# Infinidat/slimfastq

Hardware: AMD Instinct MI355X
Metric: MB/s FASTQ compressed (higher is better)
Workload: dtype u8/u32 integer; 1 GPU; synthetic 10M x 150 bp Illumina reads per GPU, full qlts+gens+recs, frozen tables (one chain per lane), -l 3; level=3, block_reads=1024, prior_step=-1, blocks_per_gpu=9766, tables=frozen, chains_per_gpu=253906, raw_bytes_per_gpu=3702038404, parallelism=1 GPU

## Files before the change

slimfastq_amd/csrc/chains.hip:

```cpp
#include "kernels.h"
#include "dev_chain.h"
#include "dev_walk.h"
#include "dev_wave.h"
#include "gen_pack_place.h"
typedef u32 __attribute__((aligned(1))) u32_any;

#define LAST_QLT 63u
#define QROW_BYTES 256u
#define B2_INIT 0x03030303u

#define QDEC_ROW 72u
__device__ __forceinline__ void qdec_store(u16* row, u32 s, u32 cum) {
    if (s) row[8 + s - 1] = (u16)cum;
    if ((s & 7u) == 0) row[s >> 3] = (u16)cum;
    if (s == 63) row[8 + 63] = 0;
}
__global__ __launch_bounds__(256) void k_qlt_frozen_rows(const u32* __restrict__ rows66, u32 q_rows, u32* __restrict__ qrows, u16* __restrict__ qdec) {
    const u32 lane = threadIdx.x & 63;
    const u32 ctx = blockIdx.x * 4 + (threadIdx.x >> 6);
    if (ctx >= q_rows) return;
    const u32* r = rows66 + (size_t)ctx * 66;
    const u32 slot = r[lane], iend = r[65];
    if (iend == 0) {
        qrows[(size_t)ctx * 64 + lane] = (lane << 10) | (1024u << 16);
// ... 904 lines not shown
            const u32 rec = s0 + sub;
            uint4 e = tab[rec & 63u];
            if (rec >= n) e.w = 0;
            const u32 last = gp_step_last(s0, n, per);
            const u32 rec_end = done + rl(inc, last), last_len = rl(len, last);
            u32 q0 = 0;
            do {
                const u32 off = q0 + piece;
                if (off < e.w) {
                    const uint4 w = load16(buf, nbytes, ((u64)e.y << 32 | e.x) + off);
                    const uint4 vm = gp_valid4(e.w - off);
                    u32 o0, o1, o2, o3, i0, i1, i2, i3;
                    const u32 f0 = gp_fold(gp_codes(w.x, vm.x, o0, i0)), f1 = gp_fold(gp_codes(w.y, vm.y, o1, i1));
                    const u32 f2 = gp_fold(gp_codes(w.z, vm.z, o2, i2)), f3 = gp_fold(gp_codes(w.w, vm.w, o3, i3));
                    illegal |= i0 | i1 | i2 | i3;
                    u32 p01 = __builtin_amdgcn_perm(f1, f0, 0x06020400u), p23 = __builtin_amdgcn_perm(f3, f2, 0x06020400u);
                    p01 |= p01 >> 12; p23 |= p23 >> 12;
                    const u32 code = __builtin_amdgcn_perm(p23, p01, 0x05040100u);
                    if (a.exc_flag && (o0 | o1 | o2 | o3)) a.exc_flag[cp.r0 + k0 + rec] = 1;
                    const GpPlace g = gp_place(e.z + off, code);
                    __hip_atomic_fetch_or(&ring[gp_ring_slot(g.d)], g.lo, __ATOMIC_RELAXED, __HIP_MEMORY_SCOPE_WAVEFRONT);
                    __hip_atomic_fetch_or(&ring[gp_ring_slot(g.d + 1u)], g.hi, __ATOMIC_RELAXED, __HIP_MEMORY_SCOPE_WAVEFRONT);
                }
                const u32 next = gp_turn_end(rec_end, last_len, q0);
                gp_wave_fence();
                if (gp_row_ready(row, next)) {
                    const u32 t = row + lane, slot = gp_ring_slot(t);
                    const u32 v = ring[slot];
                    ring[slot] = 0;
                    if (4u * t < cap) out[t] = v;
                    row += GP_ROW;
                }
                gp_wave_fence();
                q0 += 1024u;
            } while (q0 < last_len);
        }
        done += rl(inc, 63u);
    }
    {
        const u32 t = row + lane;
        if (lane < gp_tail_dwords(row, done) && 4u * t < cap) out[t] = ring[gp_ring_slot(t)];
    }
    if (lane == 0) {
        const u32 n = (done + 3u) >> 2;
        a.csz[c] = n;
        if (n > cap) atomicMax(&a.m.blocks[cp.b].status, (u32)(-SFQ_E_OVERFLOW));
    }
    if (__any(illegal != 0u) && lane == 0) atomicMax(&a.m.blocks[cp.b].status, (u32)(-SFQ_E_GENCHAR));
}
void launch_gen_encode_c(const ChainArgs& a, hipStream_t st, u32 c0, u32 c1, bool flat) {
    constexpr int T = 256;
    if (!c1 || c1 > a.geo.nchains) c1 = a.geo.nchains;
    if (c1 <= c0) return;
    if (a.flat_raw) { hipLaunchKernelGGL(k_gen_pack_raw, dim3((c1 - c0 + 3) / 4), dim3(256), 0, st, a, c0, c1); return; }
    const dim3 grid((c1 - c0 + T - 1) / T);
    if (flat) hipLaunchKernelGGL((k_gen_encode_c<T, true>), grid, dim3(T), 0, st, a, c0, c1);
    else hipLaunchKernelGGL((k_gen_encode_c<T, false>), grid, dim3(T), 0, st, a, c0, c1);
}

__device__ __forceinline__ u32 b2_pick(u32 v, LaneDecQ& rc, const u32* rcp) {
    const u32 f0 = v & 0xff, f1 = (v >> 8) & 0xff, f2 = (v >> 16) & 0xff, f3 = v >> 24;
    const u32 c1 = f0, c2 = f0 + f1, c3 = c2 + f2, tot = c3 + f3;
    u32 r;
    const u32 prob = rc.get_freq(tot, rcp[tot], r);
    const u32 b = (prob >= c1 ? 1u : 0u) + (prob >= c2 ? 1u : 0u) + (prob >= c3 ? 1u : 0u);
    const u32 cum = b == 0 ? 0u : b == 1 ? c1 : b == 2 ? c2 : c3;
    rc.decode(r, cum, (v >> (8 * b)) & 0xff);
    return b;
}
template <int THREADS>
__global__ __launch_bounds__(THREADS) void k_gen_decode_c(ChainArgs a, DecodeArgs da, u32 c0, u32 c1 ) {
    __shared__ u32 rcp[1024];
    for (u32 i = threadIdx.x; i < 1024; i += THREADS) rcp[i] = i ? rc_recip(i) : 0u;
    __syncthreads();
    const u32 c = c0 + blockIdx.x * THREADS + threadIdx.x;
    if (c >= c1) return;
    ChainPos cp = chain_pos(a, c);
    const BlockDesc* d = &a.m.blocks[cp.b];
    LaneDecQ rc; rc.init(da.streams + a.coff[c], a.csz[c], reinterpret_cast<const u8*>(a.qesc));
    const u32* rows = gen_rows_of(a, cp.b);
    const u32 alphabet = d->solid ? 0x33323130u  : 0x54474341u ;
    const u32 mask = (1u << d->gen_bits) - 1u;
    const u32 INIT = 0x007616c7u;
    const u32 r12 = rc_recip(12u);
    u32 n_next = cp.nrec ? da.slen[cp.r0] : 0u; u64 off_next = cp.nrec ? da.soff[cp.r0] : 0ull;
    if (a.seg_len) {
        const u32 ql = da.qlen[cp.r0];
        seg_range(cp, ql > n_next ? ql : n_next);
        const u64 lo = cp.sub_lo < n_next ? cp.sub_lo : n_next;
        n_next = (u32)(n_next - lo < cp.sub_len ? n_next - lo : cp.sub_len); off_next += lo;
    }
    const u8* const raw = da.streams + a.coff[c]; const u32 raw_n = a.csz[c];
    u32 racc = 0, rnb = 0, rat = 0, rbad = 0;
    for (u32 k = 0; k < cp.nrec; k++) {
        const u32 llen = n_next; const u64 off = off_next;
        if (k + 1 < cp.nrec) { n_next = da.slen[cp.r0 + k + 1]; off_next = da.soff[cp.r0 + k + 1]; }
        LaneOut32 out; out.begin(da.seq_stage + off);
        u32 last = INIT;
        if (a.flat_raw) {
            for (u32 i = 0; i < llen; i++) {
                if (rnb == 0) {
                    if (rat + 4u <= raw_n) { racc = *reinterpret_cast<const u32_any*>(raw + rat); rat += 4u; rnb = 32u; }
                    else if (rat < raw_n) { racc = raw[rat++]; rnb = 8u; }
                    else { rbad = 1; racc = 0; rnb = 32u; }
                }
                out.put((alphabet >> (8u * (racc & 3u))) & 0xffu);
                racc >>= 2; rnb -= 2u;
            }
        } else
        if (rows) {
            u32 v = rows[last & mask];
            for (u32 i = 0; i < llen; i++) {
                const uint4 cand = *reinterpret_cast<const uint4*>(rows + ((last << 2) & mask));
                rc.top_up();
                const u32 b = b2_pick(v, rc, rcp);
                out.put((alphabet >> (8 * b)) & 0xff);
                last = (last << 2) | b;
                v = b == 0 ? cand.x : b == 1 ? cand.y : b == 2 ? cand.z : cand.w;
            }
        } else if (a.flat_quads) {
            for (u32 i = 0; i < llen; i += 4u) {
                const u32 k = llen - i < 4u ? llen - i : 4u;
                rc.top_up();
                u32 r;
                const u32 S = rc.get_freq_bits(2u * k, r);
                rc.decode1(r, S, 1u);
                for (u32 j = 0; j < k; j++) out.put((alphabet >> (8u * ((S >> (2u * j)) & 3u))) & 0xffu);
            }
        } else {
            for (u32 i = 0; i < llen; i++) {
                rc.top_up();
                u32 r;
                const u32 prob = rc.get_freq(12u, r12, r);
                const u32 b = (prob >= 3u ? 1u : 0u) + (prob >= 6u ? 1u : 0u) + (prob >= 9u ? 1u : 0u);
                rc.decode1(r, 3u * b, 3u);
                out.put((alphabet >> (8 * b)) & 0xff);
            }
        }
        out.end();
    }
    if (a.flat_raw) { if (rbad || rat != raw_n || (rnb >= 8u) || racc) atomicMax(&a.m.blocks[cp.b].status, (u32)(-SFQ_E_CORRUPT)); }
    else
    if (rc.err) atomicMax(&a.m.blocks[cp.b].status, (u32)(-SFQ_E_CORRUPT));
}
void launch_gen_decode_c(const ChainArgs& a, const DecodeArgs& da, u32 c0, u32 c1, hipStream_t st) {
    constexpr int T = 256;
    if (c1 > a.geo.nchains) c1 = a.geo.nchains;
    if (c1 <= c0) return;
    hipLaunchKernelGGL(k_gen_decode_c<T>, dim3((c1 - c0 + T - 1) / T), dim3(T), 0, st, a, da, c0, c1);
}

#include "dev_rec_lane.h"
#include "dev_wave.h"

struct RecChainPos { u32 b; u64 r0; u32 nrec; };
__device__ __forceinline__ RecChainPos rec_chain_pos(const ChainArgs& a, u32 c) {
    RecChainPos p;
    p.b = c / a.rgeo.cpb;
    const u32 j = c - p.b * a.rgeo.cpb;
    const BlockDesc* d = &a.m.blocks[p.b];
    const u32 k0 = j * a.rgeo.chain_reads;
    p.nrec = k0 < d->nrec ? (d->nrec - k0 < a.rgeo.chain_reads ? d->nrec - k0 : a.rgeo.chain_reads) : 0u;
    p.r0 = d->rec0 + k0;
    return p;
}
__device__ __forceinline__ u8* rec_chain_region(const ChainArgs& a, const RecChainPos& p, u32& cap) {
    const BlockDesc* d = &a.m.blocks[p.b];
    const u64 t0 = a.m.line_off[4 * d->rec0], tc = a.m.line_off[4 * p.r0], te = a.m.line_off[4 * (p.r0 + p.nrec)];
    const u64 lo = ((tc - t0) * 3 / 2 + 3) & ~3ull, hi = ((te - t0) * 3 / 2) & ~3ull;
    cap = hi > lo ? (u32)(hi - lo) : 0u;
    return a.m.arena + d->out_off[SFQ_S_REC] + lo;
}

#define REC_HBUF 128u
#define REC_LDS_ROWS 8u
struct RecFrozenEnc {
    static constexpr bool inband = true;
    const u32* rows; LaneEnc rc;
    u8* lbuf;
    const u16* lmap; const u32* lrows;
    __device__ __forceinline__ void record(u32) {}
    __device__ __forceinline__ const u8* stage(const u8* g, u32 n, u32 k) {
        if (n + 1 > REC_HBUF) return g;
        u8* dst = lbuf + (k & 1u) * REC_HBUF;
        const u32 nw = (n + 4) / 4;
#pragma unroll 8
        for (u32 i = 0; i < nw; i++) reinterpret_cast<u32*>(dst)[i] = reinterpret_cast<const u32_any*>(g)[i];
        return dst;
    }
    __device__ __forceinline__ void put(u32 row, u32 sym) {
        const u32 slot = lmap[row];
        const u32 e = slot != 0xFFFFu ? lrows[slot * 256 + sym] : rows[(size_t)row * 256 + sym];
        rc.encode16(FZ_CUM(e), FZ_FREQ(e));
    }
    __device__ __forceinline__ void put_u(u32 row0, u64 num) { put_u_rows(*this, row0, num); }
};
struct RecCountEnc {
    static constexpr bool inband = true;
    u32* cnt; u32 kc;
    __device__ __forceinline__ void record(u32 k) { kc = k; }
    __device__ __forceinline__ const u8* stage(const u8* g, u32, u32) { return g; }
    __device__ __forceinline__ void put(u32 row, u32 sym) { atomicAdd(&cnt[(size_t)row * 256 + sym], kc >= 1u ? 1u : 0u); }
    __device__ __forceinline__ void put_u(u32 row0, u64 num) { put_u_rows(*this, row0, num); }
};
__global__ __launch_bounds__(64) void k_rec_count(ModelArgs a, u64 nrec, u64 stride, u32 run, u32 nruns, u32* cnt, const u32* flags ) {
    const u32 i = blockIdx.x * 64 + threadIdx.x;
    if (i >= nruns) return;
    if (flags && !flags[i]) return;
    const u64 r0 = (u64)i * stride;
    if (r0 >= nrec) return;
    const u32 n = (u32)(nrec - r0 < run ? nrec - r0 : run);
    RecCountEnc cd; cd.cnt = cnt + (size_t)(blockIdx.x % REC_COUNT_COPIES) * PR_REC_ROWS * 256; cd.kc = 0;
    XfEnc x_rec; x_rec.init(nullptr, 0, XF_REC_X);
    PwTab none; none.slots = nullptr; none.hdr = nullptr; none.epoch = 0;
    u32 hb; int bad;
    rec_encode_lane(a, r0, r0, n, cd, x_rec, none, hb, bad);
}
__global__ __launch_bounds__(256) void k_rec_count_sum(u32* __restrict__ cnt) {
    const u32 i = blockIdx.x * 256 + threadIdx.x;
    if (i >= PR_REC_ROWS * 256u) return;
    u32 s = 0;
#pragma unroll 8
    for (u32 k = 1; k < REC_COUNT_COPIES; k++) s += cnt[(size_t)k * PR_REC_ROWS * 256 + i];
    if (s) cnt[i] += s;
}
#define RDEC_ROW 272u
__global__ __launch_bounds__(256) void k_rec_frozen_rows(const u32* __restrict__ f, u32 nrows, u32* __restrict__ rrows, u16* __restrict__ rdec) {
    const u32 lane = threadIdx.x & 63;
    const u32 row = blockIdx.x * 4 + (threadIdx.x >> 6);
    if (row >= nrows) return;
    const uint4 fv = *reinterpret_cast<const uint4*>(f + (size_t)row * 256 + lane * 4);
    const u32 x[4] = { fv.x + 1, fv.y + 1, fv.z + 1, fv.w + 1 };
    u32 S = x[0] + x[1] + x[2] + x[3];
#pragma unroll
    for (int d = 32; d > 0; d >>= 1) S += (u32)__shfl_xor((int)S, d, 64);
    u32 g[4]; u32 sum = 0, best = 0;
#pragma unroll
    for (int j = 0; j < 4; j++) {
        g[j] = (u32)(((u64)x[j] << 16) / S); g[j] = g[j] ? g[j] : 1u;
        sum += g[j];
        const u32 key = (g[j] << 8) | (255u - (lane * 4 + j));
        best = key > best ? key : best;
    }
#pragma unroll
    for (int d = 32; d > 0; d >>= 1) {
        sum += (u32)__shfl_xor((int)sum, d, 64);
        const u32 o = (u32)__shfl_xor((int)best, d, 64); best = o > best ? o : best;
    }
    const u32 bsym = 255u - (best & 255u);
#pragma unroll
    for (int j = 0; j < 4; j++) if (lane * 4 + j == bsym) g[j] += 65536u - sum;
    const u32 mine = g[0] + g[1] + g[2] + g[3];
    u32 incl = mine;
#pragma unroll
    for (int d = 1; d < 64; d <<= 1) { const u32 o = (u32)__shfl_up((int)incl, d, 64); if (lane >= (u32)d) incl += o; }
    u32 cum = incl - mine;
    if (rdec) {
        u16* rd = rdec + (size_t)row * RDEC_ROW;
        if ((lane & 3) == 0) rd[lane >> 2] = (u16)cum;
        const u32 c1 = cum + g[0], c2 = c1 + g[1], c3 = c2 + g[2];
        *reinterpret_cast<uint2*>(rd + 16 + lane * 4) = make_uint2(cum | (c1 << 16), c2 | (c3 << 16));
    }
    uint4 e;
    e.x = cum | (g[0] << 16); cum += g[0];
    e.y = cum | (g[1] << 16); cum += g[1];
    e.z = cum | (g[2] << 16); cum += g[2];
    e.w = cum | (g[3] << 16);
    *reinterpret_cast<uint4*>(rrows + (size_t)row * 256 + lane * 4) = e;
}
__global__ __launch_bounds__(256) void k_rec_prior_freqs(const u32* __restrict__ cnt, u32 nrows, u32* __restrict__ f, u32* __restrict__ rtot) {
    const u32 lane = threadIdx.x & 63;
    const u32 row = blockIdx.x * 4 + (threadIdx.x >> 6);
    if (row >= nrows) return;
    const uint4 cv = *reinterpret_cast<const uint4*>(cnt + (size_t)row * 256 + lane * 4);
    u32 mx = max(max(cv.x, cv.y), max(cv.z, cv.w));
#pragma unroll
    for (int d = 32; d > 0; d >>= 1) { const u32 o = (u32)__shfl_xor((int)mx, d, 64); mx = o > mx ? o : mx; }
    u32 sh = 0;
    while ((((u64)mx * 14u) >> sh) > 32000u) sh++;
    uint4 fv;
    fv.x = (u32)(((u64)cv.x * 14u) >> sh); fv.y = (u32)(((u64)cv.y * 14u) >> sh); fv.z = (u32)(((u64)cv.z * 14u) >> sh); fv.w = (u32)(((u64)cv.w * 14u) >> sh);
    *reinterpret_cast<uint4*>(f + (size_t)row * 256 + lane * 4) = fv;
    u32 t = fv.x + fv.y + fv.z + fv.w;
#pragma unroll
    for (int d = 32; d > 0; d >>= 1) t += (u32)__shfl_xor((int)t, d, 64);
    if (lane == 0) rtot[row] = t;
}
#define RHR_PER ((PR_REC_ROWS + 255u) / 256u)
__global__ __launch_bounds__(256) void k_rec_hot_rows(const u32* __restrict__ rtot, u32 nrows, u32 nh, u16* __restrict__ map, u16* __restrict__ hot) {
    __shared__ u64 wmax[4];
    const u32 t = threadIdx.x, lane = t & 63, wave = t >> 6;
    u64 k[RHR_PER];
#pragma unroll
    for (u32 j = 0; j < RHR_PER; j++) {
        const u32 row = t + 256u * j;
        k[j] = row < nrows ? ((u64)rtot[row] << 11) | (2047u - row) : 0ull;
        if (row < nrows) map[row] = 0xFFFFu;
    }
    for (u32 i = 0; i < nh; i++) {
        u64 m = 0;
#pragma unroll
        for (u32 j = 0; j < RHR_PER; j++) m = k[j] > m ? k[j] : m;
#pragma unroll
        for (int d = 32; d > 0; d >>= 1) {
            const u64 o = ((u64)(u32)__shfl_xor((int)(u32)(m >> 32), d, 64) << 32) | (u32)__shfl_xor((int)(u32)m, d, 64);
            m = o > m ? o : m;
// ... 152 lines not shown
            u32 type = nw_lds(L, cur, lane, o, (int)wl, fnum, pct);
            if (type != ST_STR && !rec_number_prints_back(type, wl, L.text[cur][o][lane])) type = ST_STR;
            const u32 rr = (f + 1) * 16;
            if (type == ST_STR) {
                cd.put(rr + 0, type);
                cd.put_u(rr + 2, wl);
                for (u32 j = 0; j < wl; j++) cd.put(rr + 1, L.text[cur][o + j][lane]);
                L.fkind[f][lane] = 0;
                continue;
            }
            const u64 was = pct ? L.fvalue[f][lane] : 0;
            u64 gap;
            L.fkind[f][lane] = (type < ST_STR || type >= ST_DGT_Z) ? 1 : 2;
            L.fvalue[f][lane] = fnum;
            if (fnum < was) { gap = was - fnum; type++; }
            else gap = fnum - was;
            cd.put(rr + 0, type);
            cd.put_u(rr + 2, gap);
        }
        nf_prev = nf; cur = prv;
    }
    hdr_bytes_out = hdr_bytes;
    return true;
}
template <u32 ML>
__global__ __launch_bounds__(64) void k_rec_encode_f(ChainArgs a, u32* flags, const u32* only ) {
    __builtin_amdgcn_s_setprio(3);
    __shared__ RecFastLds<ML> L;
    const u32 lane = threadIdx.x;
    {
        const u32 c0 = blockIdx.x * 64 + lane;
        if (only && !__any(c0 < a.rgeo.nchains && only[c0] == 1)) return;
    }
    for (u32 i = lane; i < PR_REC_ROWS; i += 64) { const u32 sl = a.rmap[i]; L.map[i] = (u8)(sl < REC_LDS_ROWS ? sl : 0xFFu); }
    for (u32 i = lane; i < a.r_hot * 256; i += 64) L.rows[i] = a.rrows[(size_t)a.rhot[i >> 8] * 256 + (i & 255)];
    __syncthreads();
    const u32 c = blockIdx.x * 64 + lane;
    if (c >= a.rgeo.nchains) return;
    if (only && !only[c]) return;
    const RecChainPos cp = rec_chain_pos(a, c);
    BlockDesc* d = &a.m.blocks[cp.b];
    u32 cap = 0;
    u8* outp = rec_chain_region(a, cp, cap);
    RecFastEnc<RecFastLds<ML>> cd; cd.rows = a.rrows; cd.L = &L; cd.rc.init(outp, cap);
    u32 hdr_bytes = 0;
    if (!rec_fast_lane(a.m, L, lane, d->rec0, cp.r0, cp.nrec, cd, hdr_bytes)) { flags[c] = 1; return; }
    a.rhb[c] = hdr_bytes;
    a.csz[c] = cd.rc.finish();
    if (cd.rc.err & 2) atomicMax(&d->status, (u32)(-SFQ_E_OVERFLOW));
    if (cd.rc.err & 1) atomicMax(&d->status, (u32)(-SFQ_E_CORRUPT));
}
struct RecFastCount {
    u32* cnt; u32 kc;
    __device__ __forceinline__ void record(u32 k) { kc = k; }
    __device__ __forceinline__ void put(u32 row, u32 sym) { atomicAdd(&cnt[(size_t)row * 256 + sym], kc >= 1u ? 1u : 0u); }
    __device__ __forceinline__ void put_u(u32 row0, u64 num) { put_u_rows(*this, row0, num); }
};
__global__ __launch_bounds__(64) void k_rec_count_f(ModelArgs a, u64 nrec, u64 stride, u32 run, u32 nruns, u32* cnt, u32* flags) {
    __shared__ RecFastLds<127> L;
    const u32 lane = threadIdx.x;
    const u32 i = blockIdx.x * 64 + lane;
    if (i >= nruns) return;
    const u64 r0 = (u64)i * stride;
    if (r0 >= nrec) return;
    const u32 n = (u32)(nrec - r0 < run ? nrec - r0 : run);
    bool fits = true;
    for (u32 k = 0; k < n && fits; k++) {
        const u64 h0 = a.line_off[4 * (r0 + k)] + 1, h1 = a.line_off[4 * (r0 + k) + 1] - 1;
        const u32 len = h1 > h0 ? (u32)(h1 - h0) : 0;
        fits = len <= 127u && rf_stage(L, 0, lane, a.fq + h0, len) <= RF_NF;
    }
    if (!fits) { flags[i] = 1; return; }
    RecFastCount cd; cd.cnt = cnt + (size_t)(blockIdx.x % REC_COUNT_COPIES) * PR_REC_ROWS * 256; cd.kc = 0;
    u32 hb = 0;
    rec_fast_lane(a, L, lane, r0, r0, n, cd, hb);
}
void launch_rec_count(const ModelArgs& a, u64 nrec, u64 stride, u32 run, u32 nruns, u32* cnt, u32* flags, hipStream_t st) {
    hipLaunchKernelGGL(k_rec_count_f, dim3((nruns + 63) / 64), dim3(64), 0, st, a, nrec, stride, run, nruns, cnt, flags);
    hipLaunchKernelGGL(k_rec_count, dim3((nruns + 63) / 64), dim3(64), 0, st, a, nrec, stride, run, nruns, cnt, (const u32*)flags);
    hipLaunchKernelGGL(k_rec_count_sum, dim3((PR_REC_ROWS * 256u + 255) / 256), dim3(256), 0, st, cnt);
}
#define RT_TOK_PER_REC 40u
#define RT_STAGED 24u
template <u32 ML>
struct RecTokLds {
    static constexpr u32 maxlen = ML;
    static constexpr u32 NW = (ML + 4) / 4;
    static constexpr u32 NWP = NW | 1u;
    u32 tw[66][NWP];
    u8 off[1][RF_NF][66], wln[1][RF_NF][66], sep[1][RF_NF][66];
    u8 nf[66];
    u32 tokst[RT_STAGED][64];
    __device__ __forceinline__ u32 byte(u32 col, u32 pos) const { return reinterpret_cast<const u8*>(tw[col])[pos]; }
};
struct HdrMask {
    u64 lo, hi;
    __device__ __forceinline__ u32 count() const { return (u32)__popcll(lo) + (u32)__popcll(hi); }
    __device__ __forceinline__ u32 take() {
        if (lo) { const u32 p = (u32)__ffsll((long long)lo) - 1u; lo &= lo - 1; return p; }
        const u32 p = 63u + (u32)__ffsll((long long)hi); hi &= hi - 1; return p;
    }
};
template <typename LT>
__device__ __forceinline__ bool rt_stage(LT& L, u32 col, const u8* text, u32 n, HdrMask& M) {
    const u32_any* g = reinterpret_cast<const u32_any*>(text);
    const u32 kn = n >> 2, nw = kn + 1;
    const u32 fill = (n & 3u) == 3u ? 0u : ~0u << (8u * ((n & 3u) + 1u));
    u32 zero = 0, mw[4] = {};
#pragma unroll
    for (u32 k0 = 0; k0 < LT::NW; k0 += 4) {
        if (!__any(k0 < nw)) break;
        u32 wv[4];
#pragma unroll
        for (u32 q = 0; q < 4; q++) wv[q] = k0 + q < nw && k0 + q < LT::NW ? g[k0 + q] : ~0u;
#pragma unroll
        for (u32 q = 0; q < 4; q++) {
            const u32 k = k0 + q;
            if (k >= LT::NW) break;
            L.tw[col][k] = wv[q];
            const u32 w = wv[q] | (k == kn ? fill : 0u);
            const u32 x = w & 0x7f7f7f7fu, y = x | 0x20202020u;
            const u32 dig = (x + 0x50505050u) & ~(x + 0x46464646u);
            const u32 let = (y + 0x1f1f1f1fu) & ~(y + 0x05050505u);
            const u32 t = ~((dig | let) & ~w) & 0x80808080u;
            mw[k / 8] |= (((t >> 7) * 0x01020408u) >> 24) << (4u * (k % 8));
            zero |= ~(((w & 0x7f7f7f7fu) + 0x7f7f7f7fu) | w) & 0x80808080u;
        }
    }
    M.lo = mw[0] | ((u64)mw[1] << 32);
    M.hi = mw[2] | ((u64)mw[3] << 32);
    if (n < 63) { M.lo &= (2ull << n) - 1; M.hi = 0; }
    else if (n == 63) M.hi = 0;
    else M.hi &= (2ull << (n - 64)) - 1;
    return zero == 0;
}
template <typename LT>
__device__ __forceinline__ void rt_fields(LT& L, u32 col, HdrMask m, u32 nf) {
    u32 start = 0;
    for (u32 f = 0; f < nf; f++) {
        const u32 p = m.take();
        L.off[0][f][col] = (u8)start; L.wln[0][f][col] = (u8)(p - start); L.sep[0][f][col] = (u8)L.byte(col, p);
        start = p + 1;
    }
}
struct TokCount { u32 n; __device__ __forceinline__ void put(u32, u32) { n++; } __device__ __forceinline__ void put_u(u32 row0, u64 num) { put_u_rows(*this, row0, num); } };
struct TokStage {
    u32* p; u32 n;
    __device__ __forceinline__ void put(u32 row, u32 sym) { if (n < RT_STAGED) p[n * 64u] = (row << 8) | sym; n++; }
    __device__ __forceinline__ void put_u(u32 row0, u64 num) { put_u_rows(*this, row0, num); }
};
struct TokStore { u32* p; __device__ __forceinline__ void put(u32 row, u32 sym) { *p++ = (row << 8) | sym; } __device__ __forceinline__ void put_u(u32 row0, u64 num) { put_u_rows(*this, row0, num); } };
template <typename LT>
__device__ __forceinline__ u32 nw_tok(const LT& L, u32 col, u32 off, u32 len, u64& num) {
    u32 v = 0, lead = 0;
    bool plain = len <= 9u;
    if (plain)
        for (u32 j = 0; j < len; j++) {
            const u32 d = L.byte(col, off + j) - '0';
            plain = plain && d <= 9u;
            lead |= (j < 2u && d == 0u) ? 1u << j : 0u;
            v = v * 10u + d;
        }
    if (plain) {
        num = (lead & 3u) == 3u ? 0u : v;
        return (lead & 3u) == 3u ? ST_STR : (lead & 1u) ? ST_DGT_Z : ST_DGT;
    }
    return field_type([&](u32 j) -> u32 { return L.byte(col, off + j); }, len, num, 0);
}
template <typename LT, typename EM>
__device__ __forceinline__ bool rec_tokens(const LT& L, u32 col, u32 n, u32 nf, bool shape, u64 map, u64 since, EM& em) {
    em.put(REC_FLAG_ROW, shape ? 1u : 0u);
    if (shape) {
        em.put_u(REC_FLAG_ROW + 2, n);
        for (u32 j = 0; j < n; j++) em.put(REC_FLAG_ROW + 1, L.byte(col, j));
        return true;
    }
    em.put_u(0 * 16 + 2, map);
    for (u64 todo = map; todo; todo &= todo - 1) {
        const u32 f = (u32)__ffsll((long long)todo) - 1u;
        const u32 o = L.off[0][f][col], wl = L.wln[0][f][col];
        u64 fnum;
        u32 type = nw_tok(L, col, o, wl, fnum);
        if (type != ST_STR && !rec_number_prints_back(type, wl, L.byte(col, o))) type = ST_STR;
        if (type >= ST_HGT && type <= ST_HLTC_Z) return false;
        const u32 rr = (f + 1) * 16;
        if (type == ST_STR) {
            em.put(rr + 0, type);
            em.put_u(rr + 2, wl);
            for (u32 j = 0; j < wl; j++) em.put(rr + 1, L.byte(col, o + j));
            continue;
        }
        u64 was = 0;
        if ((since >> f) & 1) {
            const u32 po = L.off[0][f][col - 1], pwl = L.wln[0][f][col - 1];
            u64 pn;
            u32 pt = nw_tok(L, col - 1, po, pwl, pn);
            if (pt != ST_STR && !rec_number_prints_back(pt, pwl, L.byte(col - 1, po))) pt = ST_STR;
            if (pt == ST_DGT || pt == ST_DGT_Z) was = pn;
        }
        u64 gap;
        if (fnum < was) { gap = was - fnum; type++; }
        else gap = fnum - was;
        em.put(rr + 0, type);
        em.put_u(rr + 2, gap);
    }
    return true;
}
template <u32 ML>
__global__ __launch_bounds__(64) void k_rec_tokens(ChainArgs a, u32* __restrict__ tok, u32* __restrict__ ntok, u32* __restrict__ flags) {
    __shared__ RecTokLds<ML> L;
    const u32 lane = threadIdx.x, col = lane + 1;
    const u32 c = blockIdx.x;
    const RecChainPos cp = rec_chain_pos(a, c);
    if (cp.nrec == 0) { if (lane == 0) { ntok[c] = 0; a.rhb[c] = 0; } return; }
    const u64 base = a.m.blocks[cp.b].rec0;
    u32 bad = 0, base_n = 0;
    if (lane == 0) {
        const u64 h0 = a.m.line_off[4 * base] + 1, h1 = a.m.line_off[4 * base + 1] - 1;
        base_n = h1 > h0 ? (u32)(h1 - h0) : 0;
        if (base_n > ML) bad = 1;
        else {
            HdrMask m0;
            const bool ok = rt_stage(L, 0, a.m.fq + h0, base_n, m0);
            const u32 nf = m0.count();
            if (!ok || nf > RF_NF) bad = 1; else { rt_fields(L, 0, m0, nf); L.nf[0] = (u8)nf; }
        }
    }
    if (__any(bad != 0)) { if (lane == 0) flags[c] = 1; return; }
    const u64 end = cp.r0 + cp.nrec;
    const u64 first = cp.r0 == base ? cp.r0 + 1 : cp.r0;
    u32 hdr_bytes = cp.r0 == base ? rl(base_n, 0) : 0u;
    u64 since0 = 0;
    u32 total = 0;
    u32* const out = tok + cp.r0 * RT_TOK_PER_REC;
    const u32 cap = cp.nrec * RT_TOK_PER_REC;
    for (u64 rb = first; rb < end; rb += 64) {
        const u64 r = rb + lane;
        const bool valid = r < end;
        u32 n = 0, nf = 0;
        if (valid) {
            const u64 h0 = a.m.line_off[4 * r] + 1, h1 = a.m.line_off[4 * r + 1] - 1;
            n = h1 > h0 ? (u32)(h1 - h0) : 0;
            if (n > ML) bad = 1;
            else {
                HdrMask m;
                const bool ok = rt_stage(L, col, a.m.fq + h0, n, m);
                nf = m.count();
                if (!ok || nf > RF_NF) bad = 1; else { rt_fields(L, col, m, nf); L.nf[col] = (u8)nf; }
            }
        }
        if (__any(bad != 0)) { if (lane == 0) flags[c] = 1; return; }
        __syncthreads();
        bool shape = false; u64 map = 0;
        if (valid) {
            shape = nf != L.nf[col - 1];
            for (u32 f = 0; !shape && f < nf; f++) shape = L.sep[0][f][col] != L.sep[0][f][col - 1];
            if (!shape)
                for (u32 f = 0; f < nf; f++) {
                    const u32 wl = L.wln[0][f][col];
                    bool ch = wl != L.wln[0][f][col - 1];
                    if (!ch) {
                        const u32 o = L.off[0][f][col], po = L.off[0][f][col - 1];
                        for (u32 j = 0; j < wl; j++) if (L.byte(col, o + j) != L.byte(col - 1, po + j)) { ch = true; break; }
                    }
                    if (ch) map |= 1ull << f;
                }
        }
        u32 rs = shape ? 1u : 0u; u64 mm = shape ? 0ull : map;
#pragma unroll
        for (u32 dd = 1; dd < 64; dd <<= 1) {
            const u32 ors = (u32)__shfl_up((int)rs, dd, 64);
            const u64 omm = (u64)__shfl_up((unsigned long long)mm, dd, 64);
            if (lane >= dd) { mm = rs ? mm : (mm | omm); rs |= ors; }
        }
        u32 ers = (u32)__shfl_up((int)rs, 1, 64); u64 emm = (u64)__shfl_up((unsigned long long)mm, 1, 64);
        if (lane == 0) { ers = 0; emm = 0; }
        const u64 since = ers ? emm : (since0 | emm);
        {
            const u32 lrs = (u32)__shfl((int)rs, 63, 64); const u64 lmm = (u64)__shfl((unsigned long long)mm, 63, 64);
            since0 = lrs ? lmm : (since0 | lmm);
        }
        TokStage tl; tl.p = &L.tokst[0][lane]; tl.n = 0;
        bool ok = true;
        if (valid) ok = rec_tokens(L, col, n, nf, shape, map, since, tl);
        if (__any(!ok)) { if (lane == 0) flags[c] = 1; return; }
        const u32 cnt = tl.n;
        const u32 incl = wave_incl_scan(cnt);
        const u32 round = rl(incl, 63);
        if (total + round > cap) { if (lane == 0) flags[c] = 1; return; }
        u32* const dst = out + total + (incl - cnt);
        if (__any(cnt > RT_STAGED)) {
            if (valid) { TokStore ts; ts.p = dst; rec_tokens(L, col, n, nf, shape, map, since, ts); }
        } else
            for (u32 j = 0; __any(j < cnt); j++) if (j < cnt) dst[j] = L.tokst[j][lane];
        total += round;
        hdr_bytes += rl(wave_incl_scan(n), 63);
        __syncthreads();
        if (rb + 64 < end) {
            for (u32 p = lane; p < RecTokLds<ML>::NWP; p += 64) L.tw[0][p] = L.tw[64][p];
            if (lane < RF_NF) { L.off[0][lane][0] = L.off[0][lane][64]; L.wln[0][lane][0] = L.wln[0][lane][64]; L.sep[0][lane][0] = L.sep[0][lane][64]; }
            if (lane == 0) L.nf[0] = L.nf[64];
            __syncthreads();
        }
    }
    if (lane == 0) { ntok[c] = total; a.rhb[c] = hdr_bytes; }
}
#define RC_LDS_ROWS 16u
struct RecCodeLds { u32 rows[RC_LDS_ROWS * 256]; u8 map[PR_REC_ROWS]; };
__device__ __forceinline__ u32 rec_code_entry(const RecCodeLds& L, const u32* __restrict__ grows, u32 row, u32 sym) {
    const u32 slot = L.map[row];
    return slot != 0xFFu ? L.rows[slot * 256 + sym] : grows[(size_t)row * 256 + sym];
}
__global__ __launch_bounds__(256) void k_rec_code(ChainArgs a, const u32* __restrict__ tok, const u32* __restrict__ ntok, const u32* __restrict__ flags, u32 n_hot) {
    __shared__ RecCodeLds L;
    for (u32 i = threadIdx.x; i < PR_REC_ROWS; i += 256) { const u32 sl = a.rmap[i]; L.map[i] = (u8)(sl < n_hot ? sl : 0xFFu); }
    for (u32 i = threadIdx.x; i < n_hot * 256; i += 256) L.rows[i] = a.rrows[(size_t)a.rhot[i >> 8] * 256 + (i & 255)];
    __syncthreads();
    const u32 c = blockIdx.x * 256 + threadIdx.x;
    if (c >= a.rgeo.nchains || flags[c]) return;
    const RecChainPos cp = rec_chain_pos(a, c);
    BlockDesc* d = &a.m.blocks[cp.b];
    u32 cap = 0;
    u8* outp = rec_chain_region(a, cp, cap);
    RecFastEnc<RecCodeLds> cd; cd.rows = a.rrows; cd.L = &L; cd.rc.init(outp, cap);
    const uint4* t = reinterpret_cast<const uint4*>(tok + cp.r0 * RT_TOK_PER_REC);
    const u32 n = ntok[c];
    const u32* const grows = a.rrows;
#define RC_ENTRY(tk, on) rec_code_entry(L, grows, (on) ? (tk) >> 8 : 0u, (tk) & 0xffu)
#define RC_ENTRIES(v, i) make_uint4(RC_ENTRY((v).x, (i) < n), RC_ENTRY((v).y, (i) + 1 < n), RC_ENTRY((v).z, (i) + 2 < n), RC_ENTRY((v).w, (i) + 3 < n))
    constexpr u32 Q = 4;
    uint4 t1[Q], e[Q];
#pragma unroll
    for (u32 k = 0; k < Q; k++) { uint4 t0 = make_uint4(0, 0, 0, 0); t1[k] = t0; if (4 * k < n) t0 = t[k]; if (4 * (Q + k) < n) t1[k] = t[Q + k]; e[k] = RC_ENTRIES(t0, 4u * k); }
    for (u32 i = 0; i < n; i += 4 * Q) {
        uint4 t2[Q], e2[Q];
#pragma unroll
        for (u32 k = 0; k < Q; k++) { t2[k] = make_uint4(0, 0, 0, 0); if (i + 4 * (2 * Q + k) < n) t2[k] = t[(i >> 2) + 2 * Q + k]; }
#pragma unroll
        for (u32 k = 0; k < Q; k++) e2[k] = RC_ENTRIES(t1[k], i + 4u * (Q + k));
#pragma unroll
        for (u32 k = 0; k < Q; k++) {
            const u32 j = i + 4 * k;
            if (j < n) cd.rc.encode16(FZ_CUM(e[k].x), FZ_FREQ(e[k].x));
            if (j + 1 < n) cd.rc.encode16(FZ_CUM(e[k].y), FZ_FREQ(e[k].y));
            if (j + 2 < n) cd.rc.encode16(FZ_CUM(e[k].z), FZ_FREQ(e[k].z));
            if (j + 3 < n) cd.rc.encode16(FZ_CUM(e[k].w), FZ_FREQ(e[k].w));
        }
#pragma unroll
        for (u32 k = 0; k < Q; k++) { t1[k] = t2[k]; e[k] = e2[k]; }
    }
#undef RC_ENTRIES
#undef RC_ENTRY
    a.csz[c] = cd.rc.finish();
    if (cd.rc.err & 2) atomicMax(&d->status, (u32)(-SFQ_E_OVERFLOW));
    if (cd.rc.err & 1) atomicMax(&d->status, (u32)(-SFQ_E_CORRUPT));
}
void launch_rec_encode_c(const ChainArgs& a, u32* flags, u32* flags2, u32* tok, u32* ntok, u32 n_hot, u32 max_hdr, hipStream_t st, u32 min_hdr, hipEvent_t after_tokens) {
    const u32 nc = a.rgeo.nchains;
    if (!nc) return;
    if (min_hdr > 127) {
        hipLaunchKernelGGL(k_rec_encode_c, dim3((nc + 63) / 64), dim3(64), 0, st, a, (const u32*)nullptr);
        return;
    }
    if (max_hdr <= 62) hipLaunchKernelGGL(k_rec_tokens<62>, dim3(nc), dim3(64), 0, st, a, tok, ntok, flags);
    else if (max_hdr <= 94) hipLaunchKernelGGL(k_rec_tokens<94>, dim3(nc), dim3(64), 0, st, a, tok, ntok, flags);
    else hipLaunchKernelGGL(k_rec_tokens<127>, dim3(nc), dim3(64), 0, st, a, tok, ntok, flags);
    if (after_tokens) (void)hipEventRecord(after_tokens, st);
    hipLaunchKernelGGL(k_rec_code, dim3((nc + 255) / 256), dim3(256), 0, st, a, (const u32*)tok, (const u32*)ntok, (const u32*)flags, n_hot < RC_LDS_ROWS ? n_hot : RC_LDS_ROWS);
    const dim3 grid((nc + 63) / 64);
    if (max_hdr <= 62) hipLaunchKernelGGL(k_rec_encode_f<62>, grid, dim3(64), 0, st, a, flags2, (const u32*)flags);
    else if (max_hdr <= 94) hipLaunchKernelGGL(k_rec_encode_f<94>, grid, dim3(64), 0, st, a, flags2, (const u32*)flags);
    else hipLaunchKernelGGL(k_rec_encode_f<127>, grid, dim3(64), 0, st, a, flags2, (const u32*)flags);
    hipLaunchKernelGGL(k_rec_encode_c, grid, dim3(64), 0, st, a, (const u32*)flags2);
}
u64 rec_token_bytes(u64 nrec) { return nrec * RT_TOK_PER_REC * 4; }

__device__ __forceinline__ u32 chn_zz(const u32* __restrict__ csz, u32 i, u32 b1, u32 b2, u32 b3) {
    const u32 prev = (i == 0 || i == b1 || i == b2 || i == b3) ? 0u : csz[i - 1];
    const i32 d = (i32)(csz[i] - prev);
    return ((u32)d << 1) ^ (u32)(d >> 31);
}
__global__ __launch_bounds__(256) void k_chn_len(const u32* __restrict__ csz, u32 n, u32 b1, u32 b2, u32 b3, u32* __restrict__ len) {
    const u32 i = blockIdx.x * 256 + threadIdx.x;
    if (i >= n) return;
    const u32 z = chn_zz(csz, i, b1, b2, b3);
    len[i] = z < (1u << 7) ? 1u : z < (1u << 14) ? 2u : z < (1u << 21) ? 3u : z < (1u << 28) ? 4u : 5u;
}
__global__ __launch_bounds__(256) void k_chn_bytes(const u32* __restrict__ csz, u32 n, u32 b1, u32 b2, u32 b3, const u64* __restrict__ off, u8* __restrict__ out, u64* __restrict__ info) {
    const u32 i = blockIdx.x * 256 + threadIdx.x;
    if (i == 0) { info[0] = off[b2]; info[1] = off[n]; }
    if (i >= n) return;
    u32 z = chn_zz(csz, i, b1, b2, b3);
    u8* w = out + off[i];
    while (z >= 0x80u) { *w++ = (u8)(z | 0x80u); z >>= 7; }
    *w = (u8)z;
}
void launch_chain_index_bytes(const u32* csz, u32 n, u32 b1, u32 b2, u32 b3, u32* len, u64* off, u64* scan_tmp, u8* out, u64* info, hipStream_t st) {
    if (!n) return;
    hipLaunchKernelGGL(k_chn_len, dim3((n + 255) / 256), dim3(256), 0, st, csz, n, b1, b2, b3, len);
    launch_scan_u32((const u32*)len, off, n, scan_tmp, st);
    hipLaunchKernelGGL(k_chn_bytes, dim3((n + 255) / 256), dim3(256), 0, st, csz, n, b1, b2, b3, (const u64*)off, out, info);
}

typedef u32 u32x4 __attribute__((ext_vector_type(4)));
typedef const __attribute__((address_space(3))) u16* lds_row;
typedef const __attribute__((address_space(1))) u16* glb_row;
template <typename V> __device__ __forceinline__ void unpack8v(V v, u32* o) {
    o[0] = v.x & 0xffffu; o[1] = v.x >> 16; o[2] = v.y & 0xffffu; o[3] = v.y >> 16; o[4] = v.z & 0xffffu; o[5] = v.z >> 16; o[6] = v.w & 0xffffu; o[7] = v.w >> 16;
}
__device__ __forceinline__ u32x4 row16(lds_row p) { return *reinterpret_cast<const __attribute__((address_space(3))) u32x4*>(p); }
__device__ __forceinline__ u32x4 row16(glb_row p) { return *reinterpret_cast<const __attribute__((address_space(1))) u32x4*>(p); }
template <typename P>
__device__ __forceinline__ u32 rdec_search(P rd, u32 prob, u32& cum, u32& next) {
    u32 cc[16], ff[16];
    unpack8v(row16(rd), cc);
    unpack8v(row16(rd + 8), cc + 8);
    u32 k = 0;
#pragma unroll
    for (u32 j = 1; j < 16; j++) k += cc[j] <= prob;
    P fr = rd + 16 + k * 16;
    unpack8v(row16(fr), ff);
    unpack8v(row16(fr + 8), ff + 8);
    u32 s = 0;
    cum = ff[0]; next = 65536u;
#pragma unroll
    for (u32 j = 15; j >= 1; j--) next = cc[j] > prob ? cc[j] : next;
#pragma unroll
    for (u32 j = 15; j >= 1; j--) next = ff[j] > prob ? ff[j] : next;
#pragma unroll
    for (u32 j = 1; j < 16; j++) { const bool le = ff[j] <= prob; s += le; cum = le ? ff[j] : cum; }
    return k * 16 + s;
}
struct RecFrozenDec {
    static constexpr bool inband = true;
    const u16* rdec; LaneDec rc;
    __device__ __forceinline__ u32 get(u32 row) {
        const u32 prob = rc.get_freq16();
        u32 cum, next;
        const u32 s = rdec_search((glb_row)(rdec + (size_t)row * RDEC_ROW), prob, cum, next);
        rc.decode(cum, next - cum);
        return s;
    }
    __device__ __forceinline__ u64 get_u(u32 row0) { return get_u_rows(*this, row0); }
    __device__ __forceinline__ u32 err() const { return rc.err; }
};
__global__ __launch_bounds__(64) void k_rec_decode_c(ChainArgs a, DecodeArgs da, const u32* flags, u32 c0, u32 c1 ) {
    const u32 c = c0 + blockIdx.x * blockDim.x + threadIdx.x;
    if (c >= c1) return;
// ... 427 lines not shown
```

Before: 366,100 MB/s.

## Parse header numeric fields with SWAR and share previous-record values across lanes

Replaces the per-byte digit loop in header field tokenizing with a SWAR parser that reads packed words and folds up to nine digits with a few multiplies. Each lane now parses its own field once and gets the previous record's value through a wave shift and a carried cross-batch value, instead of re-parsing the neighbour's field. Field iteration follows the wave-wide OR of change masks so lanes stay converged. Varint emission is also unrolled into branchless symbol helpers. This adds DPP reductions and more complex lane-0 boundary logic, which risks subtle correctness issues.

```diff
diff --git a/slimfastq_amd/csrc/chains.hip b/slimfastq_amd/csrc/chains.hip
--- a/slimfastq_amd/csrc/chains.hip
+++ b/slimfastq_amd/csrc/chains.hip
@@ -1080,6 +1080,7 @@
 
 #include "dev_rec_lane.h"
 #include "dev_wave.h"
+#include "rec_digits.h"
 
 struct RecChainPos { u32 b; u64 r0; u32 nrec; };
 __device__ __forceinline__ RecChainPos rec_chain_pos(const ChainArgs& a, u32 c) {
@@ -1538,59 +1539,93 @@
 struct TokStore { u32* p; __device__ __forceinline__ void put(u32 row, u32 sym) { *p++ = (row << 8) | sym; } __device__ __forceinline__ void put_u(u32 row0, u64 num) { put_u_rows(*this, row0, num); } };
 template <typename LT>
 __device__ __forceinline__ u32 nw_tok(const LT& L, u32 col, u32 off, u32 len, u64& num) {
-    u32 v = 0, lead = 0;
-    bool plain = len <= 9u;
-    if (plain)
-        for (u32 j = 0; j < len; j++) {
-            const u32 d = L.byte(col, off + j) - '0';
-            plain = plain && d <= 9u;
-            lead |= (j < 2u && d == 0u) ? 1u << j : 0u;
-            v = v * 10u + d;
-        }
-    if (plain) {
-        num = (lead & 3u) == 3u ? 0u : v;
-        return (lead & 3u) == 3u ? ST_STR : (lead & 1u) ? ST_DGT_Z : ST_DGT;
-    }
-    return field_type([&](u32 j) -> u32 { return L.byte(col, off + j); }, len, num, 0);
+    const RdField r = rd_parse9(L.tw[col], off, len);
+    if (len <= 9u && r.plain) {
+        const bool str = r.lead == 3u || len == 0u;
+        num = str ? 0u : r.value;
+        return str ? ST_STR : (r.lead & 1u) ? ST_DGT_Z : ST_DGT;
+    }
+    u32 type = field_type([&](u32 j) -> u32 { return L.byte(col, off + j); }, len, num, 0);
+    if (type != ST_STR && !rec_number_prints_back(type, len, L.byte(col, off))) type = ST_STR;
+    return type;
+}
+template <typename EM>
+__device__ __forceinline__ void tok_put_u(EM& em, u32 row0, u64 num) {
+    const u32 n = rd_u_count(num);
+    em.put(row0, rd_u_sym0(n, num));
+    if (n >= 2u) em.put(row0 + 1, rd_u_sym1(n, num));
+    if (n >= 6u) {
+        const u32 r = row0 + (n == 6u ? 2u : 6u), lo = (u32)num;
+        em.put(r, lo & 0xffu); em.put(r + 1, (lo >> 8) & 0xffu); em.put(r + 2, (lo >> 16) & 0xffu); em.put(r + 3, lo >> 24);
+    }
+    if (n == 10u) {
+        const u32 hi = (u32)(num >> 32);
+#pragma nounroll
+        for (u32 j = 0; j < 4; j++) em.put(row0 + 10 + j, (hi >> (8 * j)) & 0xffu);
+    }
+}
+__device__ __forceinline__ u32 wave_or(u32 x) {
+    x |= (u32)__builtin_amdgcn_update_dpp(0, (int)x, DPP_ROW_SHR(1), 0xf, 0xf, false);
+    x |= (u32)__builtin_amdgcn_update_dpp(0, (int)x, DPP_ROW_SHR(2), 0xf, 0xf, false);
+    x |= (u32)__builtin_amdgcn_update_dpp(0, (int)x, DPP_ROW_SHR(4), 0xf, 0xf, false);
+    x |= (u32)__builtin_amdgcn_update_dpp(0, (int)x, DPP_ROW_SHR(8), 0xf, 0xf, false);
+    x |= (u32)__builtin_amdgcn_update_dpp(0, (int)x, DPP_ROW_BCAST15, 0xa, 0xf, false);
+    x |= (u32)__builtin_amdgcn_update_dpp(0, (int)x, DPP_ROW_BCAST31, 0xc, 0xf, false);
+    return rl(x, 63);
 }
 template <typename LT, typename EM>
-__device__ __forceinline__ bool rec_tokens(const LT& L, u32 col, u32 n, u32 nf, bool shape, u64 map, u64 since, EM& em) {
-    em.put(REC_FLAG_ROW, shape ? 1u : 0u);
-    if (shape) {
-        em.put_u(REC_FLAG_ROW + 2, n);
-        for (u32 j = 0; j < n; j++) em.put(REC_FLAG_ROW + 1, L.byte(col, j));
-        return true;
-    }
-    em.put_u(0 * 16 + 2, map);
-    for (u64 todo = map; todo; todo &= todo - 1) {
-        const u32 f = (u32)__ffsll((long long)todo) - 1u;
-        const u32 o = L.off[0][f][col], wl = L.wln[0][f][col];
-        u64 fnum;
-        u32 type = nw_tok(L, col, o, wl, fnum);
-        if (type != ST_STR && !rec_number_prints_back(type, wl, L.byte(col, o))) type = ST_STR;
-        if (type >= ST_HGT && type <= ST_HLTC_Z) return false;
-        const u32 rr = (f + 1) * 16;
-        if (type == ST_STR) {
-            em.put(rr + 0, type);
-            em.put_u(rr + 2, wl);
-            for (u32 j = 0; j < wl; j++) em.put(rr + 1, L.byte(col, o + j));
-            continue;
-        }
-        u64 was = 0;
-        if ((since >> f) & 1) {
-            const u32 po = L.off[0][f][col - 1], pwl = L.wln[0][f][col - 1];
-            u64 pn;
-            u32 pt = nw_tok(L, col - 1, po, pwl, pn);
-            if (pt != ST_STR && !rec_number_prints_back(pt, pwl, L.byte(col - 1, po))) pt = ST_STR;
-            if (pt == ST_DGT || pt == ST_DGT_Z) was = pn;
-        }
-        u64 gap;
-        if (fnum < was) { gap = was - fnum; type++; }
-        else gap = fnum - was;
-        em.put(rr + 0, type);
-        em.put_u(rr + 2, gap);
-    }
-    return true;
+__device__ __forceinline__ bool rec_tokens(const LT& L, u64 cw_in, u32 kept_in, u64& cw_out, u32 lane, bool valid, u32 n, u32 nf, bool shape,
+                                           u32 map, u32 since, u32 orm, u32 need, EM& em) {
+    const u32 col = lane + 1;
+    if (valid) {
+        em.put(REC_FLAG_ROW, shape ? 1u : 0u);
+        if (shape) {
+            tok_put_u(em, REC_FLAG_ROW + 2, n);
+            for (u32 j = 0; j < n; j++) em.put(REC_FLAG_ROW + 1, L.byte(col, j));
+        } else tok_put_u(em, 0 * 16 + 2, map);
+    }
+    bool ok = true;
+    for (u32 todo = orm; todo; todo &= todo - 1) {
+        const u32 f = (u32)__ffs((int)todo) - 1u;
+        const bool own = (map >> f) & 1u, parse = (need >> f) & 1u;
+        const bool want_was = own && ((since >> f) & 1u);
+        const bool kept = (kept_in >> f) & 1u;
+        const bool left0 = want_was && lane == 0 && !kept;
+        u32 type = ST_STR, o = 0, wl = 0;
+        u64 fnum = 0, give = 0, was0 = 0;
+#pragma nounroll
+        for (u32 turn = __any(left0) ? 0u : 1u; turn < 2u; turn++) {
+            const u32 pc = turn ? col : 0u;
+            if (turn ? parse : left0) {
+                o = L.off[0][f][pc]; wl = L.wln[0][f][pc];
+                type = nw_tok(L, pc, o, wl, fnum);
+                give = (type == ST_DGT || type == ST_DGT_Z) ? fnum : 0ull;
+            }
+            if (!turn) was0 = give;
+        }
+        const u32 g_lo = (u32)give, g_hi = (u32)(give >> 32);
+        const u64 last = (u64)rl(g_lo, 63) | ((u64)rl(g_hi, 63) << 32), before = (u64)rl((u32)cw_in, f) | ((u64)rl((u32)(cw_in >> 32), f) << 32);
+        if (lane == f) cw_out = last;
+        u64 was = (u64)wave_shr1(g_lo, 0u) | ((u64)wave_shr1(g_hi, 0u) << 32);
+        if (lane == 0) was = kept ? before : was0;
+        if (!want_was) was = 0;
+        if (own) {
+            const u32 rr = (f + 1) * 16;
+            if (type >= ST_HGT && type <= ST_HLTC_Z) ok = false;
+            else if (type == ST_STR) {
+                em.put(rr + 0, type);
+                tok_put_u(em, rr + 2, wl);
+                for (u32 j = 0; j < wl; j++) em.put(rr + 1, L.byte(col, o + j));
+            } else {
+                u64 gap;
+                if (fnum < was) { gap = was - fnum; type++; }
+                else gap = fnum - was;
+                em.put(rr + 0, type);
+                tok_put_u(em, rr + 2, gap);
+            }
+        }
+    }
+    return ok;
 }
 template <u32 ML>
 __global__ __launch_bounds__(64) void k_rec_tokens(ChainArgs a, u32* __restrict__ tok, u32* __restrict__ ntok, u32* __restrict__ flags) {
@@ -1618,6 +1653,7 @@
     u32 hdr_bytes = cp.r0 == base ? rl(base_n, 0) : 0u;
     u64 since0 = 0;
     u32 total = 0;
+    u32 kept = 0; u64 cw = 0;
     u32* const out = tok + cp.r0 * RT_TOK_PER_REC;
     const u32 cap = cp.nrec * RT_TOK_PER_REC;
     for (u64 rb = first; rb < end; rb += 64) {
@@ -1666,9 +1702,13 @@
             const u32 lrs = (u32)__shfl((int)rs, 63, 64); const u64 lmm = (u64)__shfl((unsigned long long)mm, 63, 64);
             since0 = lrs ? lmm : (since0 | lmm);
         }
+        const u32 map32 = (u32)map, since32 = (u32)since;
+        const u32 orm = wave_or(map32);
+        u32 need = map32 | wave_shl1(map32 & since32, 0u);
+        if (lane == 63 && valid) need |= orm & ((1u << nf) - 1u);
+        u64 cw_out = 0;
         TokStage tl; tl.p = &L.tokst[0][lane]; tl.n = 0;
-        bool ok = true;
-        if (valid) ok = rec_tokens(L, col, n, nf, shape, map, since, tl);
+        const bool ok = rec_tokens(L, cw, kept, cw_out, lane, valid, n, nf, shape, map32, since32, orm, need, tl);
         if (__any(!ok)) { if (lane == 0) flags[c] = 1; return; }
         const u32 cnt = tl.n;
         const u32 incl = wave_incl_scan(cnt);
@@ -1676,10 +1716,12 @@
         if (total + round > cap) { if (lane == 0) flags[c] = 1; return; }
         u32* const dst = out + total + (incl - cnt);
         if (__any(cnt > RT_STAGED)) {
-            if (valid) { TokStore ts; ts.p = dst; rec_tokens(L, col, n, nf, shape, map, since, ts); }
+            TokStore ts; ts.p = dst;
+            rec_tokens(L, cw, kept, cw_out, lane, valid, n, nf, shape, map32, since32, orm, need, ts);
         } else
             for (u32 j = 0; __any(j < cnt); j++) if (j < cnt) dst[j] = L.tokst[j][lane];
         total += round;
+        kept = rl(need, 63); cw = cw_out;
         hdr_bytes += rl(wave_incl_scan(n), 63);
         __syncthreads();
         if (rb + 64 < end) {
diff --git a/slimfastq_amd/csrc/rec_digits.h b/slimfastq_amd/csrc/rec_digits.h
--- /dev/null
+++ b/slimfastq_amd/csrc/rec_digits.h
@@ -0,0 +1,36 @@
+#pragma once
+#include "dev_common.h"
+
+struct RdField {
+    u32 value;
+    u32 plain;
+    u32 lead;
+};
+__device__ __forceinline__ u32 rd_not_digit(u32 y) { return (((y & 0x7f7f7f7fu) + 0x76767676u) | y) & 0x80808080u; }
+__device__ __forceinline__ u32 rd_fold4(u32 y) {
+    const u32 t = (y * 10u + (y >> 8)) & 0x00ff00ffu;
+    return (t * 100u + (t >> 16)) & 0xffffu;
+}
+__device__ __forceinline__ u32 rd_funnel(u32 hi, u32 lo, u32 sh) { return (u32)(((((u64)hi) << 32) | lo) >> sh); }
+__device__ __forceinline__ RdField rd_parse9(const u32* tw, u32 off, u32 len) {
+    const u32 last = off + len - 1u;
+    const u32 q = len && last >= 4u ? last >> 2 : 0u;
+    const u32 sh = 8u * ((last & 3u) + 1u);
+    const u32 x2 = tw[q], x1 = tw[q >= 1u ? q - 1u : 0u], x0 = tw[q >= 2u ? q - 2u : 0u];
+    const u32 m2 = len >= 4u ? ~0u : len ? ~0u << (8u * (4u - len)) : 0u;
+    const u32 m1 = len >= 8u ? ~0u : len > 4u ? ~0u << (8u * (8u - len)) : 0u;
+    const u32 y2 = (rd_funnel(x2, x1, sh) ^ 0x30303030u) & m2;
+    const u32 y1 = (rd_funnel(x1, x0, sh) ^ 0x30303030u) & m1;
+    const u32 y0 = len == 9u ? ((x0 >> (sh - 8u)) & 0xffu) ^ 0x30u : 0u;
+    RdField r;
+    r.plain = (rd_not_digit(y2) | rd_not_digit(y1)) == 0u && y0 <= 9u ? 1u : 0u;
+    r.value = y0 * 100000000u + rd_fold4(y1) * 10000u + rd_fold4(y2);
+    const u64 y21 = ((u64)y2 << 32) | y1;
+    const u32 nz = y0 ? 0u : y21 ? 1u + ((u32)__builtin_ctzll(y21) >> 3) : 9u;
+    r.lead = (nz + len >= 10u ? 1u : 0u) | (nz + len >= 11u ? 2u : 0u);
+    return r;
+}
+
+__device__ __forceinline__ u32 rd_u_count(u64 num) { return num <= 0x7fu ? 1u : num < 0x7ffeu ? 2u : num < (1ull << 32) ? 6u : 10u; }
+__device__ __forceinline__ u32 rd_u_sym0(u32 n, u64 num) { return n == 1u ? (u32)num : n == 2u ? (0x80u | (u32)(num >> 8)) & 0xffu : 0xffu; }
+__device__ __forceinline__ u32 rd_u_sym1(u32 n, u64 num) { return n == 2u ? (u32)num & 0xffu : n == 6u ? 0xfeu : 0xffu; }
```

Result: faster. 372,600 MB/s, median of 6 (+1.8%).
